# nanoporetech/bonito

Hardware: AMD Instinct MI355X
Metric: signal samples/sec/GPU (chunk=10000, batch=512) + read accuracy vs ref (higher is better)
Workload: dtype f16

## Files before the change

bonito_amd/_lib.py:

```python
import ctypes as C
import os

_HERE = os.path.dirname(os.path.abspath(__file__))
LIB_PATH = os.environ.get("BONITO_HIP_LIB") or os.path.join(_HERE, "libbonito_hip.so")


class HipEngineError(RuntimeError):
    """An entry point of libbonito_hip.so reported an error."""


class bh_layer_t(C.Structure):
    _fields_ = [
        ("kind", C.c_int32), ("in_size", C.c_int32), ("out_size", C.c_int32),
        ("winlen", C.c_int32), ("stride", C.c_int32), ("padding", C.c_int32),
        ("activation", C.c_int32), ("reverse", C.c_int32),
        ("nhead", C.c_int32), ("dim_ff", C.c_int32), ("win_left", C.c_int32), ("win_right", C.c_int32),
        ("scale_factor", C.c_int32), ("groups", C.c_int32), ("add_residual", C.c_int32), ("quantize", C.c_int32), ("reserved_i", C.c_int32 * 1),
        ("scale", C.c_float), ("clamp_lo", C.c_float), ("clamp_hi", C.c_float),
        ("blank_score", C.c_float), ("alpha", C.c_float), ("eps", C.c_float), ("reserved_f", C.c_float * 2),
        ("w0", C.c_void_p), ("b0", C.c_void_p), ("w1", C.c_void_p), ("b1", C.c_void_p),
        ("w2", C.c_void_p), ("w3", C.c_void_p), ("w4", C.c_void_p), ("w5", C.c_void_p),
    ]


BH_ACT = {None: 0, "none": 0, "swish": 1, "tanh": 2, "relu": 3}
BH_LAYER_CONV, BH_LAYER_LSTM, BH_LAYER_LINEAR_CRF, BH_LAYER_CLAMP = 1, 2, 3, 4
BH_LAYER_TRANSFORMER, BH_LAYER_UPSAMPLE, BH_LAYER_TCS_BLOCK, BH_LAYER_CTC_DECODER = 5, 6, 7, 8
BH_LAYER_DWCONV, BH_LAYER_RESIDUAL_PROJ, BH_LAYER_LINEAR = 9, 10, 11

_vp, _i, _f, _l, _sz = C.c_void_p, C.c_int, C.c_float, C.c_long, C.c_size_t

SIGNATURES = {
    "bh_last_error": (C.c_char_p, []),
    "bh_abi_version": (_i, []),
    "bh_sizeof_layer": (_sz, []),
    "bh_device_count": (_i, []),
    "bh_encoder_create": (_i, [C.POINTER(bh_layer_t), _i, _i, _i, _i, C.POINTER(_vp)]),
    "bh_encoder_destroy": (None, [_vp]),
    "bh_encoder_output_shape": (_i, [_vp, _i, C.POINTER(_i), C.POINTER(_i), C.POINTER(_i)]),
    "bh_encoder_forward": (_i, [_vp, _vp, _i, _i, _vp, _vp]),
    "bh_encoder_check": (_i, [_vp, _vp]),
    "bh_encoder_error_flag": (_i, [_vp]),
    "bh_encoder_last_ticket": (_l, [_vp]),
    "bh_encoder_error_flag_at": (_i, [_vp, _l]),
    "bh_encoder_ack": (_i, [_vp, _l]),
    "bh_encoder_describe": (_i, [_vp, C.c_char_p, _sz]),
    "bh_encoder_profile": (_i, [_vp, _i]),
    "bh_encoder_profile_read": (_i, [_vp, C.POINTER(C.c_float), C.POINTER(_i)]),
    "bh_crf_viterbi_workspace": (_sz, [_i, _i, _i]),
    "bh_crf_viterbi": (_i, [_vp, _i, _i, _i, _i, _f, _l, _l, _vp, _vp, _vp, _vp, _vp]),
    "bh_crf_reverse_complement": (_i, [_vp, _vp, _i, _i, _i, _i, _l, _l, _vp]),
    "bh_crf_logz": (_i, [_vp, _i, _i, _i, _f, _vp, _vp, _vp]),
    "bh_crf_seq_workspace": (_sz, [_i, _i, _i, _i]),
    "bh_crf_seq_logz": (_i, [_vp, _i, _i, _i, _i, _f, _l, _l, _vp, _i, _i, _vp, _vp, _vp, _vp]),
    "bh_crf_seq_viterbi": (_i, [_vp, _i, _i, _i, _i, _f, _l, _l, _vp, _i, _i, _vp, _vp, _vp, _vp, _vp]),
    "bh_crf_seq_logz_free": (_i, [_vp, _i, _i, _i, _f, _l, _l, _vp, _i, _i, _vp, _vp, _vp, _vp]),
    "bh_crf_logz_dense": (_i, [_vp, _i, _i, _i, _i, _f, _l, _l, _vp, _vp]),
    "bh_crf_seq_grad_workspace": (_sz, [_i, _i, _i, _i]),
    "bh_crf_seq_logz_grad": (_i, [_vp, _i, _i, _i, _i, _f, _l, _l, _vp, _i, _i, _vp, _vp, _vp, _vp, _vp, _l, _l, _i, _i, _vp]),
    "bh_crf_logz_dense_grad_workspace": (_sz, [_i, _i, _i]),
    "bh_crf_logz_dense_grad": (_i, [_vp, _i, _i, _i, _i, _f, _l, _l, _vp, _vp, _vp, _vp, _l, _l, _i, _vp]),
    "bh_sw_workspace": (_sz, [_i, _i, _i]),
    "bh_sw_align": (_i, [_vp, _l, _vp, _vp, _l, _vp, _i, _i, _i, _i, _i, _vp, _sz, _vp, _vp, _l, _vp, _vp]),
    "bh_sg_align": (_i, [_vp, _l, _vp, _vp, _l, _vp, _i, _i, _i, _i, _i, _vp, _sz, _vp, _vp, _l, _vp, _vp]),
    "bh_nw_workspace": (_sz, [_i, _i, _i, _l]),
    "bh_nw_align": (_i, [_vp, _l, _vp, _vp, _l, _vp, _i, _i, _vp, _sz, _vp, _vp, _l, _vp, _vp]),
    "bh_set_option": (_i, [C.c_char_p, _i]),
    "bh_signal_normalise": (_i, [_vp, _vp, _vp, _vp, _i, _i, C.c_double, C.c_double, C.c_double, C.c_double, C.c_double, C.c_double,
                            _i, _vp, _vp, _vp, _vp, _vp]),
    "bh_signal_chunks": (_i, [_vp, _vp, _vp, _vp, _vp, _vp, _vp, _vp, _vp, _vp, _i, _i, _vp, _vp]),
    "bh_crf_posterior_viterbi_workspace": (_sz, [_i, _i, _i]),
    "bh_crf_posterior_viterbi": (_i, [_vp, _i, _i, _i, _f, _vp, _vp, _vp, _vp]),
    "bh_beam_search_workspace": (_sz, [_i, _i, _i]),
    "bh_beam_search": (_i, [_vp, _i, _i, _i, _i, _f, _f, _f, _f, _vp, _vp, _vp, _vp, _vp, _vp]),
    "bh_beam_search_plan": (_i, [_i, _i, _i, _i, _i, C.POINTER(C.c_int32), _i]),
    "bh_linear": (_i, [_vp, _vp, _vp, _vp, _i, _i, _i, _i, _i, _i, _i, _f, _f, _f, _i, _i, _l, _l, _i, _vp]),
    "bh_linear_residual": (_i, [_vp, _vp, _vp, _vp, _i, _i, _i, _i, _i, _i, _i, _f, _f, _f, _i, _i, _l, _l, _i, _vp, _i, _f, _vp]),
    "bh_linear_qkv_rotary": (_i, [_vp, _vp, _vp, _vp, _i, _i, _i, _vp, _i, _f, _vp]),
    "bh_linear_last_kernel": (_i, []),
    "bh_conv1d_first": (_i, [_vp, _vp, _vp, _vp, _i, _i, _i, _i, _i, _i, _i, _f, _f, _l, _l, _vp]),
    "bh_conv1d_packed_halves": (_sz, [_i, _i, _i]),
    "bh_conv1d_pack": (_i, [_vp, _i, _i, _i, _vp]),
    "bh_conv1d": (_i, [_vp, _vp, _vp, _vp, _i, _i, _i, _i, _i, _i, _i, _i, _f, _f, _l, _l, _vp]),
    "bh_conv1d_front3": (_i, [_vp, _i, _i, _vp, _vp, _i, _i, _i, _f, _f, _vp, _vp, _i, _i, _i, _f, _f, _vp, _vp, _i, _i, _i, _i, _i, _f, _f,
                              _vp, _l, _l, _vp]),
    "bh_conv1d_last_kernel": (_i, []),
    "bh_ctc_greedy_decode": (_i, [_vp, _vp, _i, _i, _f, _f, _vp, _vp, _vp, _vp, _vp]),
    "bh_ctc_beam_search_workspace": (_sz, [_l, _i, _i, _i]),
    "bh_ctc_beam_search": (_i, [_vp, _vp, _i, _i, _i, _f, _vp, _vp, _vp, _vp, _vp]),
    "bh_dwconv1d": (_i, [_vp, _vp, _vp, _i, _i, _i, _i, _i, _i, _vp]),
    "bh_rotary_table": (_i, [_i, _i, _vp]),
    "bh_attention": (_i, [_vp, _vp, _vp, _i, _i, _i, _i, _i, _i, _vp]),
    "bh_attention_prerotated": (_i, [_vp, _vp, _i, _i, _i, _i, _i, _i, _vp]),
    "bh_rmsnorm_residual": (_i, [_vp, _vp, _vp, _vp, _l, _i, _f, _f, _vp]),
    "bh_lstm_pack_whh": (_i, [_vp, _i, _vp]),
    "bh_host_compact": (_l, [_vp, _l, _vp]),
    "bh_host_chunk_rows": (_l, [_vp, _l, _i, _i, _l, _l, _vp]),
    "bh_host_format_read": (_l, [_vp, _vp, _vp, _vp, _i, _l, _l, _i, _i, _i, _i, _i, _i, C.c_double, C.c_char_p, C.c_char_p, _l, _l,
                                 _vp, _l, _vp, _vp]),
    "bh_host_mean_qscore": (C.c_double, [C.c_char_p, _l]),
    "bh_host_svb16_decode": (_l, [_vp, _l, _l, _vp]),
    "bh_lstm_workspace": (_sz, [_i, _i]),
    "bh_lstm_layer": (_i, [_vp, _vp, _vp, _i, _i, _i, _i, _vp, _vp, _i, _vp]),
    "bh_lstm_q8_layer": (_i, [_vp, _f, _vp, _vp, _vp, _i, _i, _i, _i, _i, _vp, _vp, _vp, _vp]),
    "bh_lstm_layer_family": (_i, [_vp, _vp, _vp, _vp, _i, _i, _i, _i, _i, _i, _vp, _vp]),
    "bh_lstm_launch_plan": (_i, [_i, _i, _i, _i, _i, C.POINTER(C.c_int32), _i]),
    "bh_encoder_debug_read": (_i, [_vp, _vp, _sz, _sz]),
    "bh_encoder_set_option": (_i, [_vp, C.c_char_p, _i]),
}

_lib = None


CONV_KERNELS = {"none": 0, "first": 1, "ws_384": 20, "ws_96": 21, "front3_384": 30, "front3_96": 31, "dwconv": 40, "igemm_base": 100}


def conv_igemm_code(ntt, fs):
    return CONV_KERNELS["igemm_base"] + 10 * ntt + int(fs)


LSTM_FAMILIES = {"wave": 0, "fused": 1, "stream": 2, "wgx": 3, "wgx2": 4, "cta": 5, "wide": 6, "q8": 7}


def lib():
    global _lib
    if _lib is None:
        if not os.path.exists(LIB_PATH):
            raise HipEngineError(
                "%s not found: the MI355X engine is not built (run `python build.py`). "
                "bonito_amd has no CPU fallback." % LIB_PATH
            )
        import torch
        handle = C.CDLL(LIB_PATH)
        for name, (res, args) in SIGNATURES.items():
            fn = getattr(handle, name)
            fn.restype = res
            fn.argtypes = args
        if handle.bh_sizeof_layer() != C.sizeof(bh_layer_t):
            raise HipEngineError("bh_layer_t layout mismatch between include/bonito_hip.h and bonito_amd/_lib.py")
        _lib = handle
    return _lib


def last_error():
    msg = lib().bh_last_error()
    return msg.decode() if msg else ""


def check(rc, what=""):
    if rc != 0:
        raise HipEngineError("%s failed (rc=%d): %s" % (what or "libbonito_hip call", rc, last_error()))


def stream_ptr(device=None):
    import torch
    return C.c_void_p(torch.cuda.current_stream(device).cuda_stream)


def ptr(t):
    if t is None:
        return None
    return C.c_void_p(t.data_ptr())
```

bonito_amd/csrc/gemm.hip:

```cpp
#include <type_traits>
#include "common.h"
#include "kernels.h"
#include "options.h"

namespace bh {

struct GemmArgs {
    const half_t* X;
    const half_t* W;
    const float* bias;
    const half_t* res;
    int ldres;
    float res_scale = 1.0f;
    half_t* out;
    int M, N, K;
    int ldx, ldw, ldo;
    float scale;
    float clamp_lo, clamp_hi;
    int row_div;
    long row_s_hi, row_s_lo;
    int row_lim;
    int n_ft, n_tt;
    int stagger = 0;
    const float* rot_cs = nullptr;
// ... 766 lines not shown
                        for (int r = 0; r < 4; ++r) {
                            x[tt][t][r] = lo[r] * cc[r] - hi[r] * ss[r];
                            x[tt][t + 2][r] = hi[r] * cc[r] + lo[r] * ss[r];
                        }
                    }
                }
            }
        }
        if constexpr (ACT != ACT_NONE) {
#pragma unroll
            for (int tt = 0; tt < 2; ++tt)
#pragma unroll
                for (int jj = 0; jj < 4; ++jj)
#pragma unroll
                    for (int r = 0; r < 4; ++r) x[tt][jj][r] = apply_act<ACT>(x[tt][jj][r]);
        }
        if constexpr (!plain) {
#pragma unroll
            for (int tt = 0; tt < 2; ++tt)
#pragma unroll
                for (int jj = 0; jj < 4; ++jj)
#pragma unroll
                    for (int r = 0; r < 4; ++r) x[tt][jj][r] = fminf(fmaxf(x[tt][jj][r] * p.scale, p.clamp_lo), p.clamp_hi);
        }
#pragma unroll
        for (int tt = 0; tt < 2; ++tt) {
            const int r = 16 * tt + c16, sw = (c16 >> 1) & 7;
#pragma unroll
            for (int jj = 0; jj < 4; ++jj)
                *(uint2_t*)(base + r * 128 + (((2 * jj + (g >> 1)) ^ sw) << 4) + 8 * (g & 1)) =
                    __builtin_bit_cast(uint2_t, __builtin_convertvector(x[tt][jj], half4_t));
        }
    };
    auto blocks = [&](auto masked, auto with_bias) {
        constexpr bool MASKED = decltype(masked)::value;
        write_block(0, with_bias);
#pragma unroll
        for (int b = 0; b < 8; ++b) {
            const int i = b >> 1, P = b & 1;
            uint4_t o[4];
#pragma unroll
            for (int rr = 0; rr < 4; ++rr) {
                const int row = tl + 8 * rr;
                o[rr] = *(const uint4_t*)(scratch + (b & 1) * 4096 + row * 128 + ((q ^ ((row >> 1) & 7)) << 4));
            }
            if (b + 1 < 8) write_block(b + 1, with_bias);
#pragma unroll
            for (int rr = 0; rr < 4; ++rr) {
                const int u = 4 * b + rr;
                const bool live = !MASKED || tw + 32 * i + 8 * rr + tl < mlim;
                if constexpr (!MASKED) { if (u >= W4_NOW16) park[u - W4_NOW16] = o[rr]; }
                if ((!MASKED && u < W4_NOW16) || (MASKED && live))
                    __builtin_amdgcn_raw_buffer_store_b128(o[rr], orsrc, ovoff + P * 128 + (32 * i + 8 * rr) * rowbytes, 0, 0);
            }
        }
    };
    if (tw + 128 <= mlim) {
        if (p.bias != nullptr) blocks(std::false_type{}, std::true_type{});
        else blocks(std::false_type{}, std::false_type{});
        return true;
    }
    blocks(std::true_type{}, std::true_type{});
    return false;
}

template <bool GATED, bool T16, typename PARK, int NP>
__device__ __forceinline__ void w4_store_parked(const PARK (&park)[NP], const W4Store& st) {
    const __amdgpu_buffer_rsrc_t rsrc = __builtin_amdgcn_make_buffer_rsrc(
        (void*)(((unsigned long long)st.srd[1] << 32) | st.srd[0]), 0, 0x7ffffff0, 0x00020000);
    if constexpr (GATED && T16) {
#pragma unroll
        for (int idx = 0; idx < NP; ++idx) __builtin_amdgcn_raw_buffer_store_b128(park[idx], rsrc, st.voff + w4_store_rowg(idx) * st.rowb, 0, 0);
        return;
    } else {
#pragma unroll
    for (int idx = 0; idx < NP; ++idx) {
        const int row = T16 ? w4_store_row16(idx) : w4_store_row(idx), col = T16 ? w4_store_col16(idx) : w4_store_col(idx);
        if constexpr (GATED) __builtin_amdgcn_raw_buffer_store_b64(park[idx], rsrc, st.voff + col * 64 + row * st.rowb, 0, 0);
        else __builtin_amdgcn_raw_buffer_store_b128(park[idx], rsrc, st.voff + col * 128 + row * st.rowb, 0, 0);
    }
    }
}

template <int IDX0, int S, bool WIDE, bool FIRST, typename PARK>
__device__ __forceinline__ void w4_inst_st(float16_t (&acc)[4][4], half8_t (&fa)[2][4], half8_t (&fb)[2][4], const unsigned (&rab)[4],
                                           const unsigned (&rbb)[4], unsigned sa, unsigned sb, unsigned san, unsigned sbn, const unsigned (&vd1)[8],
                                           const unsigned (&vd2)[8], const char* sd1, const char* sd2, unsigned md1, unsigned md2, unsigned,
                                           const PARK (&park)[W4_NPARK], const W4Store& st, std::false_type) {
    if constexpr (S == 4 && WIDE && !FIRST) gemm_ktile_st4w<IDX0>(acc, fa, fb, rab, rbb, sa, sb, san, sbn, vd1, vd2, sd1, sd2, md1, md2, park, st.srd, st.voff, st.rowb);
    else if constexpr (S == 4 && WIDE && FIRST) gemm_ktile_first_st4w<IDX0>(acc, fa, fb, rab, rbb, sa, sb, san, sbn, vd1, vd2, sd1, sd2, md1, md2, park, st.srd, st.voff, st.rowb);
    else if constexpr (S == 4 && !WIDE && !FIRST) gemm_ktile_st4n<IDX0>(acc, fa, fb, rab, rbb, sa, sb, san, sbn, vd1, vd2, sd1, sd2, md1, md2, park, st.srd, st.voff, st.rowb);
    else if constexpr (S == 4 && !WIDE && FIRST) gemm_ktile_first_st4n<IDX0>(acc, fa, fb, rab, rbb, sa, sb, san, sbn, vd1, vd2, sd1, sd2, md1, md2, park, st.srd, st.voff, st.rowb);
    else static_assert(S == 4, "tools/gen_gemmstep.py emits the four-stores-per-instance variants only");
}

template <int IDX0, int S, bool WIDE, bool FIRST>
__device__ __forceinline__ void w4_inst_st(float4_t (&acc)[8][8], half8_t (&fa)[8], half8_t (&fb)[2][8], const unsigned (&rab)[2],
                                           const unsigned (&rbb)[2], unsigned sa, unsigned sb, unsigned san, unsigned sbn, const unsigned (&vd1)[8],
                                           const unsigned (&vd2)[8], const char* sd1, const char* sd2, unsigned md1, unsigned md2, unsigned wv,
                                           const uint4_t (&park)[W4_NPARKG], const W4Store& st, std::true_type ) {
    static_assert(S == 4, "tools/gen_gemmstep.py emits the four-stores-per-instance variants only");
    if constexpr (!FIRST) gemm_ktile16_st4g<IDX0>(acc, fa, fb, rab, rbb, sa, sb, san, sbn, vd1, vd2, sd1, sd2, md1, md2, wv, park, st.srd, st.voff, st.rowb);
    else gemm_ktile16_first_st4g<IDX0>(acc, fa, fb, rab, rbb, sa, sb, san, sbn, vd1, vd2, sd1, sd2, md1, md2, wv, park, st.srd, st.voff, st.rowb);
}
template <int IDX0, int S, bool WIDE, bool FIRST, typename PARK>
__device__ __forceinline__ void w4_inst_st(float4_t (&acc)[8][8], half8_t (&fa)[8], half8_t (&fb)[2][8], const unsigned (&rab)[2],
                                           const unsigned (&rbb)[2], unsigned sa, unsigned sb, unsigned san, unsigned sbn, const unsigned (&vd1)[8],
                                           const unsigned (&vd2)[8], const char* sd1, const char* sd2, unsigned md1, unsigned md2, unsigned wv,
                                           const PARK (&park)[W4_NPARK16], const W4Store& st, std::false_type) {
    if constexpr (S == 4 && WIDE && !FIRST) gemm_ktile16_st4w<IDX0>(acc, fa, fb, rab, rbb, sa, sb, san, sbn, vd1, vd2, sd1, sd2, md1, md2, wv, park, st.srd, st.voff, st.rowb);
    else if constexpr (S == 4 && WIDE && FIRST) gemm_ktile16_first_st4w<IDX0>(acc, fa, fb, rab, rbb, sa, sb, san, sbn, vd1, vd2, sd1, sd2, md1, md2, wv, park, st.srd, st.voff, st.rowb);
    else if constexpr (S == 4 && !WIDE && !FIRST) gemm_ktile16_st4n<IDX0>(acc, fa, fb, rab, rbb, sa, sb, san, sbn, vd1, vd2, sd1, sd2, md1, md2, wv, park, st.srd, st.voff, st.rowb);
    else if constexpr (S == 4 && !WIDE && FIRST) gemm_ktile16_first_st4n<IDX0>(acc, fa, fb, rab, rbb, sa, sb, san, sbn, vd1, vd2, sd1, sd2, md1, md2, wv, park, st.srd, st.voff, st.rowb);
    else static_assert(S == 4, "tools/gen_gemmstep.py emits the four-stores-per-instance variants only");
}

__device__ __forceinline__ void w4_settle(float16_t (&acc)[4][4]) {
    asm volatile("s_nop 7\n\ts_nop 7\n\ts_nop 3"
                 : "+a"(acc[0][0]), "+a"(acc[0][1]), "+a"(acc[0][2]), "+a"(acc[0][3]), "+a"(acc[1][0]), "+a"(acc[1][1]), "+a"(acc[1][2]),
                   "+a"(acc[1][3]), "+a"(acc[2][0]), "+a"(acc[2][1]), "+a"(acc[2][2]), "+a"(acc[2][3]), "+a"(acc[3][0]), "+a"(acc[3][1]),
                   "+a"(acc[3][2]), "+a"(acc[3][3]));
}
__device__ __forceinline__ void w4_settle(float4_t (&acc)[8][8]) {
#define W4_ROW(i) "+a"(acc[i][0]), "+a"(acc[i][1]), "+a"(acc[i][2]), "+a"(acc[i][3]), "+a"(acc[i][4]), "+a"(acc[i][5]), "+a"(acc[i][6]), "+a"(acc[i][7])
    asm volatile("s_nop 7\n\ts_nop 7\n\ts_nop 3" : W4_ROW(0), W4_ROW(1), W4_ROW(2), W4_ROW(3), W4_ROW(4), W4_ROW(5), W4_ROW(6), W4_ROW(7));
#undef W4_ROW
}
__device__ __forceinline__ void w4_ktile(float16_t (&acc)[4][4], half8_t (&fa)[2][4], half8_t (&fb)[2][4], const unsigned (&rab)[4], const unsigned (&rbb)[4],
                                         unsigned sa, unsigned sb, unsigned san, unsigned sbn, const unsigned (&vd1)[8], const unsigned (&vd2)[8],
                                         const char* sd1, const char* sd2, unsigned md1, unsigned md2, unsigned, bool first) {
    if (first) gemm_ktile_first(acc, fa, fb, rab, rbb, sa, sb, san, sbn, vd1, vd2, sd1, sd2, md1, md2);
    else gemm_ktile(acc, fa, fb, rab, rbb, sa, sb, san, sbn, vd1, vd2, sd1, sd2, md1, md2);
}
__device__ __forceinline__ void w4_ktile(float4_t (&acc)[8][8], half8_t (&fa)[8], half8_t (&fb)[2][8], const unsigned (&rab)[2], const unsigned (&rbb)[2],
                                         unsigned sa, unsigned sb, unsigned san, unsigned sbn, const unsigned (&vd1)[8], const unsigned (&vd2)[8],
                                         const char* sd1, const char* sd2, unsigned md1, unsigned md2, unsigned wv, bool first) {
    if (first) gemm_ktile16_first(acc, fa, fb, rab, rbb, sa, sb, san, sbn, vd1, vd2, sd1, sd2, md1, md2, wv);
    else gemm_ktile16(acc, fa, fb, rab, rbb, sa, sb, san, sbn, vd1, vd2, sd1, sd2, md1, md2, wv);
}

template <int ACT, bool GATED, int S, int MODE, bool T16 = false>
__global__ __launch_bounds__(256, 1) void gemm_w4_kernel(GemmArgs p) {
    extern __shared__ __attribute__((aligned(16))) char smem[];
    const int tid = threadIdx.x;
    const int lane = tid & 63;
    const int wave = __builtin_amdgcn_readfirstlane(tid >> 6);
    const int wa = wave >> 1, wb = wave & 1;
    const int nk = p.K / 64;

    unsigned rab[T16 ? 2 : 4], rbb[T16 ? 2 : 4];
    if constexpr (T16) {
        const int row = lane & 15, kg = lane >> 4, g = (row >> 1) & 7;
#pragma unroll
        for (int sl = 0; sl < 2; ++sl) {
            const unsigned off = (unsigned)(row * 128 + (((4 * sl + kg) ^ g) << 4));
            rab[sl] = wa * 16384 + off;
            rbb[sl] = wb * 16384 + off;
        }
    } else {
        const int row = lane & 31, hh = lane >> 5, g = (row >> 1) & 7;
#pragma unroll
        for (int ks = 0; ks < 4; ++ks) {
            const unsigned off = (unsigned)(row * 128 + (((2 * ks + hh) ^ g) << 4));
            rab[ks] = wa * 16384 + off;
            rbb[ks] = wb * 16384 + off;
        }
    }
    const unsigned wdma = wave * 8192;
    const char* const Ab = (const char*)p.X;
    const char* const Bb = (const char*)p.W;

    const int GF = p.w4_gf, GT = 32 / GF;
    const int tq = p.n_tt >> 3, tr = p.n_tt & 7;
    const int nbt = ((tq + (tr ? 1 : 0)) + GT - 1) / GT, nfg = (p.n_ft + GF - 1) / GF;
    const int slots = 8 * nfg * nbt * 32;
    auto tile_of = [&](int w, int& f0, int& t0) -> bool {
        const int xcd = w & 7, loc = w >> 3;
        const int NT = tq + (xcd < tr ? 1 : 0), tlo = xcd * tq + min(xcd, tr);
        const int blk = loc >> 5, within = loc & 31;
        const int fg = p.w4_order ? blk % nfg : blk / nbt, tg = p.w4_order ? blk / nfg : blk - fg * nbt;
        const int tf = fg * GF + within % GF, tt = tg * GT + within / GF;
        f0 = tf * 256;
        t0 = (tlo + tt) * 256;
        return tf < p.n_ft && tt < NT;
    };
    auto next_valid = [&](int w, int& f0, int& t0) -> int {
        for (; w < slots; w += gridDim.x)
            if (tile_of(w, f0, t0)) return w;
        return slots;
    };

    int f0 = 0, t0 = 0;
    int work = next_valid(blockIdx.x, f0, t0);
    if (work >= slots) return;
    if (p.stagger > 0) {
        const unsigned long long until = __builtin_readcyclecounter() + (unsigned long long)(((blockIdx.x >> 3) & 7) * p.stagger);
        while (__builtin_readcyclecounter() < until) __builtin_amdgcn_s_sleep(32);
    }
    unsigned va[8], vb[8];
    w4_offsets<T16>(p, f0, t0, wave, lane, va, vb);

    unsigned a0 = 0, a1 = W4_OP, a2 = 2 * W4_OP;
    unsigned b0 = W4_BRING, b1 = W4_BRING + W4_OP;
#pragma unroll
    for (int n = 0; n < 8; ++n) w4_dma(a0 + wdma + n * 1024, va[n], Ab);
#pragma unroll
    for (int n = 0; n < 8; ++n) w4_dma(b0 + wdma + n * 1024, vb[n], Bb);
#pragma unroll
    for (int n = 0; n < 8; ++n) w4_dma(a1 + wdma + n * 1024, va[n], Ab + 128);
#pragma unroll
    for (int n = 0; n < 8; ++n) w4_dma(b1 + wdma + n * 1024, vb[n], Bb + 128);
    asm volatile("s_waitcnt vmcnt(16)\n\ts_barrier" ::: "memory");
    std::conditional_t<T16, half8_t[8], half8_t[2][4]> fa;
    std::conditional_t<T16, half8_t[2][8], half8_t[2][4]> fb;
    if constexpr (T16) {
        asm volatile("ds_read_b128 %0, %10 offset:0\n\tds_read_b128 %1, %10 offset:2048\n\t"
                     "ds_read_b128 %2, %11 offset:0\n\tds_read_b128 %3, %11 offset:2048\n\tds_read_b128 %4, %11 offset:4096\n\tds_read_b128 %5, %11 offset:6144\n\t"
                     "ds_read_b128 %6, %11 offset:8192\n\tds_read_b128 %7, %11 offset:10240\n\tds_read_b128 %8, %11 offset:12288\n\tds_read_b128 %9, %11 offset:14336\n\t"
                     "s_waitcnt lgkmcnt(0)"
                     : "=&v"(fa[0]), "=&v"(fa[1]), "=&v"(fb[0][0]), "=&v"(fb[0][1]), "=&v"(fb[0][2]), "=&v"(fb[0][3]), "=&v"(fb[0][4]), "=&v"(fb[0][5]),
                       "=&v"(fb[0][6]), "=&v"(fb[0][7])
                     : "v"(rab[0] + a0), "v"(rbb[0] + b0)
                     : "memory");
    } else {
    asm volatile("ds_read_b128 %0, %8 offset:0\n\tds_read_b128 %1, %8 offset:4096\n\tds_read_b128 %2, %8 offset:8192\n\tds_read_b128 %3, %8 offset:12288\n\t"
                 "ds_read_b128 %4, %9 offset:0\n\tds_read_b128 %5, %9 offset:4096\n\tds_read_b128 %6, %9 offset:8192\n\tds_read_b128 %7, %9 offset:12288\n\t"
                 "s_waitcnt lgkmcnt(0)"
                 : "=&v"(fa[0][0]), "=&v"(fa[0][1]), "=&v"(fa[0][2]), "=&v"(fa[0][3]),
                   "=&v"(fb[0][0]), "=&v"(fb[0][1]), "=&v"(fb[0][2]), "=&v"(fb[0][3])
                 : "v"(rab[0] + a0), "v"(rbb[0] + b0)
                 : "memory");
    }

#ifdef BH_GEMM_STATS
    unsigned long long st_loop = 0, st_epi = 0, st_tiles = 0;
    const unsigned long long st_t0 = __builtin_readcyclecounter(), st_r0 = __builtin_amdgcn_s_memrealtime();
#endif
    constexpr bool G16 = GATED && T16;
    using park_t = std::conditional_t<GATED && !T16, uint2_t, uint4_t>;
    constexpr int NPARK = G16 ? W4_NPARKG : T16 ? W4_NPARK16 : W4_NPARK;
    constexpr int NST = (NPARK + S - 1) / S;
    park_t park[NPARK];
    W4Store pst;
    bool parked = false;
    const char* dA = Ab + 256;
    const char* dB = Bb + 256;
    while (true) {
#ifdef BH_GEMM_STATS
        const unsigned long long st_a = __builtin_readcyclecounter();
#endif
        int nf0 = f0, nt0 = t0;
        int tf0 = 0, tt0 = 0;
        const int next = next_valid(work + gridDim.x, tf0, tt0);
        if (next < slots) { nf0 = tf0; nt0 = tt0; }
        std::conditional_t<T16, float4_t[8][8], float16_t[4][4]> acc;
#define W4_ROTATE() do { const unsigned ta = a0; a0 = a1; a1 = a2; a2 = ta; const unsigned tb = b0; b0 = b1; b1 = tb; dA += 128; dB += 128; } while (0)
#define W4_CURSOR(k) do { if ((k) == nk - 2) { int lc = lane; asm volatile("" : "+v"(lc));  \
                                               w4_offsets<T16>(p, nf0, nt0, wave, lc, va, vb); dA = Ab; dB = Bb; } } while (0)
#define W4_ARGS acc, fa, fb, rab, rbb, a0, b0, a1, b1, va, vb, dA, dB, a2 + wdma, b0 + wdma, (unsigned)wave
        if (parked) {
#define W4_ST(T) if constexpr ((T) < NST) { W4_CURSOR(T); w4_inst_st<(T) * S, S, !GATED, (T) == 0>(W4_ARGS, park, pst, std::bool_constant<G16>{}); W4_ROTATE(); }
            W4_ST(0) W4_ST(1) W4_ST(2) W4_ST(3) W4_ST(4) W4_ST(5) W4_ST(6) W4_ST(7)
#undef W4_ST
            for (int k = NST; k < nk; ++k) {
                W4_CURSOR(k);
                w4_ktile(W4_ARGS, false);
                W4_ROTATE();
            }
        } else {
            w4_ktile(W4_ARGS, true);
            W4_ROTATE();
            for (int k = 1; k < nk; ++k) {
                W4_CURSOR(k);
                w4_ktile(W4_ARGS, false);
                W4_ROTATE();
            }
        }
#undef W4_ARGS
#undef W4_CURSOR
#undef W4_ROTATE
#ifdef BH_GEMM_STATS
        const unsigned long long st_b = __builtin_readcyclecounter();
#endif
        w4_settle(acc);
        if constexpr (G16) parked = w4_epilogue16g(p, acc, f0, t0, wa, wb, lane, smem + a2 + wdma, park, pst);
        else if constexpr (T16 && (MODE & 1) == 0) parked = w4_epilogue16p<ACT, MODE>(p, acc, f0, t0, wa, wb, lane, smem + a2 + wdma, park, pst);
        else parked = w4_epilogue<ACT, GATED, MODE>(p, acc, f0, t0, wa, wb, lane, smem + a2 + wdma, park, pst);
#ifdef BH_GEMM_STATS
        st_loop += st_b - st_a; st_epi += __builtin_readcyclecounter() - st_b; ++st_tiles;
#endif
        if (next >= slots) break;
        work = next; f0 = nf0; t0 = nt0;
    }
    if (parked) w4_store_parked<GATED, T16>(park, pst);
    asm volatile("s_waitcnt vmcnt(0)" ::: "memory");
#ifdef BH_GEMM_STATS
    if (p.dbg != nullptr && tid == 0 && (blockIdx.x == 0 || blockIdx.x == 133)) {
        unsigned long long* d = p.dbg + (blockIdx.x == 0 ? 0 : 8);
        d[0] = st_loop; d[1] = st_epi; d[2] = __builtin_readcyclecounter() - st_t0; d[3] = __builtin_amdgcn_s_memrealtime() - st_r0; d[4] = st_tiles;
    }
#endif
}

#ifdef BH_GEMM_STATS
unsigned long long* g_gemm_dbg = nullptr;
#endif
static int g_last_kernel = 0;

enum GemmKernel : int { GEMM_V1 = 1, GEMM_V2 = 2, GEMM_V3 = 3, GEMM_W4_T32 = 5, GEMM_W4_T16 = 6 };
enum GemmPath : int {
    PATH_AUTO = 0,
    PATH_V1_ONLY = 1,
    PATH_NO_256 = 2,
    PATH_NO_W4 = 3,
    PATH_FORCE_W4 = 5
};

#define W4_INSTANCES(X)                                                                                                  \
    X(ACT_NONE, true, 0)                                                                                                 \
    X(ACT_NONE, false, 0) X(ACT_NONE, false, 1) X(ACT_NONE, false, 2) X(ACT_NONE, false, 4)                              \
    X(ACT_TANH, false, 4) X(ACT_TANH, false, 0)                                                                          \
    X(ACT_SWISH, false, 0)
constexpr int w4_key(int act, bool gated, int mode) { return (act << 4) | (gated ? 8 : 0) | mode; }
static int w4_mode(const GemmArgs& a) {
    const bool plain = a.scale == 1.0f && a.clamp_lo == -INFINITY && a.clamp_hi == INFINITY;
    return (a.res != nullptr ? 1 : 0) | (a.rot_cs != nullptr ? 2 : 0) | (plain ? 0 : 4);
}
static bool w4_has_instance(int act, bool gated, int mode) {
    switch (w4_key(act, gated, mode)) {
#define W4_CASE(A_, G_, MODE_) case w4_key(A_, G_, MODE_):
        W4_INSTANCES(W4_CASE)
#undef W4_CASE
        return true;
    }
    return false;
}

static bool enough_tiles_256(const GemmArgs& a) { return (long)((a.N + BF3 - 1) / BF3) * ((a.M + BT3 - 1) / BT3) >= 512; }
static bool offsets_fit_256(const GemmArgs& a) { return (long)a.M * a.ldx < (1l << 31) && (long)a.N * a.ldw < (1l << 31); }
static bool shape_allows_w4(const GemmArgs& a) {
    return a.K % 128 == 0 && a.K >= 384
           && a.N % 256 == 0
           && ((a.row_div == 1 && a.row_s_hi == 1) || a.row_div % 256 == 0)
           && (a.rot_cs == nullptr || a.rot_T >= 256)
           && (long)a.ldo * 2 * (a.row_div == 1 ? 1 : a.row_s_lo) < (1l << 24)
           && offsets_fit_256(a);
}
static bool shape_allows_v3(const GemmArgs& a) {
    return a.K % BK3 == 0
           && a.N >= 256 && a.N % 16 == 0
           && offsets_fit_256(a);
}
static bool shape_allows_v2(const GemmArgs& a) { return a.K % BK2 == 0; }

static bool path_permits(int path, GemmKernel family) {
    switch (family) {
        case GEMM_W4_T32: case GEMM_W4_T16: return path == PATH_AUTO || path == PATH_FORCE_W4;
        case GEMM_V3: return path == PATH_AUTO || path == PATH_NO_W4;
        case GEMM_V2: return path != PATH_V1_ONLY;
        default: return true;
    }
}

struct GemmPlan {
    GemmKernel kernel;
    int grid, block, lds;
    int mode;
    GemmArgs args;
};
static GemmPlan gemm_plan(const GemmArgs& a, int act, bool gated, const Options& opt, int cus) {
    GemmPlan p;
    p.args = a;
    p.mode = w4_mode(a);
    const int path = opt.gemm_path;
    const bool w4 = shape_allows_w4(a) && (enough_tiles_256(a) || path == PATH_FORCE_W4) && path_permits(path, GEMM_W4_T16) &&
                    w4_has_instance(act, gated, p.mode);
    const bool v3 = !w4 && shape_allows_v3(a) && enough_tiles_256(a) && path_permits(path, GEMM_V3);
    if (!w4 && !v3) {
        p.kernel = shape_allows_v2(a) && path_permits(path, GEMM_V2) ? GEMM_V2 : GEMM_V1;
        p.grid = a.n_ft * a.n_tt; p.block = 256; p.lds = p.kernel == GEMM_V2 ? 4 * TILE2 : 4 * TILE_BYTES;
        return p;
    }
    const int nf = (a.N + BF3 - 1) / BF3, nt = (a.M + BT3 - 1) / BT3;
    p.args.n_ft = nf; p.args.n_tt = nt;
    if (v3) {
        p.kernel = GEMM_V3;
        p.args.stagger = opt.gemm_stagger;
        p.grid = nf * nt < cus ? nf * nt : cus; p.block = 512; p.lds = 4 * TILE3;
        return p;
    }
    p.kernel = opt.gemm_tile16 ? GEMM_W4_T16 : GEMM_W4_T32;
    p.args.stagger = opt.gemm_stagger > 0 ? opt.gemm_stagger * 256 : 0;
    p.args.w4_order = opt.gemm_order;
    int gf = 4;
    if (opt.gemm_gf > 0) for (gf = 32; gf > opt.gemm_gf;) gf >>= 1;
    while (gf > 1 && (gf > nf || (opt.gemm_gf <= 0 && nf % gf != 0))) gf >>= 1;
    p.args.w4_gf = gf;
    const int gt = 32 / gf, ntx = (nt >> 3) + ((nt & 7) ? 1 : 0);
    const long slots = 8l * ((nf + gf - 1) / gf) * ((ntx + gt - 1) / gt) * 32;
    p.grid = slots < cus ? (int)slots : cus; p.block = 256; p.lds = W4_LDS;
    return p;
}

template <int ACT, bool GATED, int MODE, bool T16>
static int launch_w4_instance(const GemmPlan& p, hipStream_t s) {
    BH_CHECK_HIP(bh_max_lds((const void*)gemm_w4_kernel<ACT, GATED, 4, MODE, T16>, p.lds));
    hipLaunchKernelGGL((gemm_w4_kernel<ACT, GATED, 4, MODE, T16>), dim3(p.grid), dim3(p.block), p.lds, s, p.args);
    return 0;
}
template <int ACT, bool GATED>
static int launch_w4(const GemmPlan& p, hipStream_t s) {
    switch (w4_key(ACT, GATED, p.mode)) {
#define W4_CASE(A_, G_, MODE_)                                                                                                   \
    case w4_key(A_, G_, MODE_):                                                                                                  \
        if constexpr (ACT == A_ && GATED == G_)                                                                                  \
            return p.kernel == GEMM_W4_T16 ? launch_w4_instance<ACT, GATED, MODE_, true>(p, s) : launch_w4_instance<ACT, GATED, MODE_, false>(p, s); \
        break;
        W4_INSTANCES(W4_CASE)
#undef W4_CASE
    }
    BH_REQUIRE(false, "linear: gemm_w4_kernel has no instance for activation %d, gated %d, mode %d", ACT, (int)GATED, p.mode);
}

template <int ACT, bool GATED>
static int launch(const GemmArgs& a, hipStream_t s) {
    const GemmPlan p = gemm_plan(a, ACT, GATED, g_opt, bh_cu_count());
    switch (p.kernel) {
        case GEMM_W4_T32: case GEMM_W4_T16:
            if (int rc = launch_w4<ACT, GATED>(p, s)) return rc;
            break;
        case GEMM_V3:
            BH_CHECK_HIP(bh_max_lds((const void*)gemm_big_kernel<ACT, GATED>, p.lds));
            hipLaunchKernelGGL((gemm_big_kernel<ACT, GATED>), dim3(p.grid), dim3(p.block), p.lds, s, p.args);
            break;
        case GEMM_V2:
            hipLaunchKernelGGL((gemm_glds_kernel<ACT, GATED>), dim3(p.grid), dim3(p.block), p.lds, s, p.args);
            break;
        case GEMM_V1:
            hipLaunchKernelGGL((gemm_kernel<ACT, GATED>), dim3(p.grid), dim3(p.block), p.lds, s, p.args);
            break;
    }
    g_last_kernel = p.kernel;
    return 0;
}

static GemmArgs gemm_args(const void* X, const void* W, const float* bias, void* out, int M, int N, int K, int ldx, int ldw, int ldo) {
    GemmArgs a;
    a.X = (const half_t*)X; a.W = (const half_t*)W; a.bias = bias; a.out = (half_t*)out;
    a.res = nullptr; a.ldres = 0;
    a.M = M; a.N = N; a.K = K; a.ldx = ldx; a.ldw = ldw; a.ldo = ldo;
    a.scale = 1.0f; a.clamp_lo = -INFINITY; a.clamp_hi = INFINITY;
    a.row_div = 1; a.row_s_hi = 1; a.row_s_lo = 0; a.row_lim = 0x7fffffff;
    a.n_ft = (N + BF - 1) / BF; a.n_tt = (M + BT - 1) / BT;
#ifdef BH_GEMM_STATS
    a.dbg = g_gemm_dbg;
#endif
    return a;
}

}

int bh_k_linear_last_kernel() { return bh::g_last_kernel; }

int bh_k_linear(const void* X, const void* W, const float* bias, void* out, int M, int N, int K,
                int ldx, int ldw, int ldo, int act, float scale, float clamp_lo, float clamp_hi,
                int gated, int row_div, long row_s_hi, long row_s_lo, int row_lim, hipStream_t stream,
                const void* residual, int ldres, float res_scale) {
    using namespace bh;
    BH_REQUIRE(M > 0 && N > 0 && K > 0, "linear: empty problem M=%d N=%d K=%d", M, N, K);
    BH_REQUIRE(K % 8 == 0 && ldx % 8 == 0 && ldw % 8 == 0, "linear: K/ldx/ldw must be multiples of 8 halves");
    BH_REQUIRE(ldo % 8 == 0, "linear: ldo must be a multiple of 8 halves");
    BH_REQUIRE(!gated || (N % 16 == 0), "linear: gated epilogue needs N %% 16 == 0");
    BH_REQUIRE(residual == nullptr || ldres % 8 == 0, "linear: ldres must be a multiple of 8 halves");
    GemmArgs a = gemm_args(X, W, bias, out, M, N, K, ldx, ldw, ldo);
    a.res = (const half_t*)residual; a.ldres = ldres; a.res_scale = res_scale;
    a.scale = scale; a.clamp_lo = clamp_lo; a.clamp_hi = clamp_hi;
    if (row_div > 0) {
        a.row_div = row_div; a.row_s_hi = row_s_hi; a.row_s_lo = row_s_lo;
        if (row_lim > 0) a.row_lim = row_lim;
    }
    int rc = 0;
    if (gated) { rc = launch<ACT_NONE, true>(a, stream); }
    else switch (act) {
        case ACT_NONE: rc = launch<ACT_NONE, false>(a, stream); break;
        case ACT_SWISH: rc = launch<ACT_SWISH, false>(a, stream); break;
        case ACT_TANH: rc = launch<ACT_TANH, false>(a, stream); break;
        case ACT_RELU: rc = launch<ACT_RELU, false>(a, stream); break;
        default: BH_REQUIRE(false, "linear: unknown activation %d", act);
    }
    if (rc) return rc;
    BH_CHECK_HIP(hipGetLastError());
    return 0;
}

int bh_k_linear_qkv_rotary(const void* X, const void* W, const float* bias, void* out, int M, int D, int K, const float* cos_sin,
                           int T, float qscale, hipStream_t stream) {
    using namespace bh;
    BH_REQUIRE(M > 0 && D > 0 && K > 0 && T > 0 && cos_sin != nullptr, "linear_qkv_rotary: bad arguments");
    BH_REQUIRE(D % 64 == 0 && K % 8 == 0, "linear_qkv_rotary: d_model must be a multiple of 64 (heads of 64), K of 8");
    GemmArgs a = gemm_args(X, W, bias, out, M, 3 * D, K, K, K, 3 * D);
    a.rot_cs = cos_sin; a.rot_T = T; a.rot_nfeat = 2 * D; a.rot_qfeat = D; a.rot_qscale = qscale;
    if (int rc = launch<ACT_NONE, false>(a, stream)) return rc;
    BH_CHECK_HIP(hipGetLastError());
    return 0;
}
```

bonito_amd/csrc/options.cpp:

```cpp
#include "options.h"

#include <string.h>

namespace bh {

Options g_opt;

#define BH_OPT(name) #name, &Options::name
static constexpr OptionRow OPTION_TABLE[] = {
    {BH_OPT(gemm_path), 0, Norm::keep, "linear GEMM kernel families: 0 auto, 1 = v1 only, 2 = no 256-tile kernel, 3 = no four-wave kernel, 5 = four-wave wherever legal"},
    {BH_OPT(gemm_tile16), 1, Norm::flag, "four-wave GEMM K-tile stream: 1 = 16x16x32 MFMAs, 0 = 32x32x16 (agree to fp16 rounding)"},
    {BH_OPT(gemm_order), 1, Norm::flag, "four-wave GEMM work order in an XCD: 1 = feature groups fastest, 0 = token blocks fastest (same bytes)"},
    {BH_OPT(gemm_gf), 0, Norm::keep, "four-wave GEMM feature tiles per block: 0 automatic, else rounded down to 1 / 2 / 4 / 8 / 16 / 32 (same bytes)"},
    {BH_OPT(gemm_stagger), 0, Norm::keep, "start-phase stagger of the persistent GEMM kernels, 0 = off (same bytes; measured without effect)"},
    {BH_OPT(attn_waves), 0, Norm::keep, "ring attention waves per workgroup: 0 automatic, 8, 12 (same results)"},
    {BH_OPT(attn_version), 2, Norm::one_or_two, "ring attention kernel: 2 = current, 1 = the first ring kernel"},
    {BH_OPT(attn_expt), 0, Norm::keep, "timing experiments of the ring attention kernel (bit mask): RESULTS ARE WRONG ON PURPOSE unless 0"},
    {BH_OPT(beam_fork), -1, Norm::keep, "posterior scan next to the beam kernel on a helper stream: -1 auto, 0 never, 1 always"},
    {BH_OPT(beam_select), 0, Norm::keep, "beam top-W selection: 0 histogram + boundary ranking, 1 radix search (same beams)"},
    {BH_OPT(beam_fuse), -1, Norm::keep, "forward / posterior scan as a second wave of the beam kernel: -1 auto (<= 256 states), 0 never, 1 always"},
    {BH_OPT(beam_cpw), 0, Norm::keep, "chunks per workgroup of the fused beam kernel at 256 states: 0 automatic, 1, 2, 4 (same bytes)"},
    {BH_OPT(decode_nt), 0, Norm::keep, "non-temporal score loads in the decode scans: 0 off"},
    {BH_OPT(viterbi_quad), 1, Norm::keep, "CRF Viterbi: 1 = four states per thread where the layout allows, 0 = the one-state kernel everywhere"},
    {BH_OPT(conv_ws), 1, Norm::keep, "weight-stationary kernel for the 384- / 96-channel 19-tap convolution: 1 on, 0 = generic implicit GEMM"},
    {BH_OPT(conv_fs), 1, Norm::keep, "feature-split instances of the implicit-GEMM convolution: 1 on, 0 = position-split"},
    {BH_OPT(conv_fuse), 1, Norm::keep, "conv1 -> conv2 -> conv3 as one kernel: 1 = 384-channel stacks, 2 = also 96-channel, 0 = three kernels"},
    {BH_OPT(conv_lds_kb), 64, Norm::positive_or_def, "KiB of LDS a workgroup of the implicit-GEMM convolution may take for its input span"},
    {BH_OPT(conv_front_pipe), 1, Norm::keep, "fused front end of the 384-channel stacks: 1 = conv1 / conv2 of the next block beside conv3 (12-wave pipeline), 0 = phase after phase (same bytes)"},
    {BH_OPT(conv_front_wgs), 0, Norm::keep, "workgroups of the pipelined front end: 0 = one per CU, n > 0 caps the grid (same bytes; test hook, A/B)"},
    {BH_OPT(lstm_max_spins), 1000000, Norm::nonneg_or_def, "bound of the recurrent kernels' exchange spin loops (0: the first incomplete poll round is a timeout)"},
    {BH_OPT(lstm_q8_variant), 0, Norm::keep, "geometry of the 8-bit recurrent kernel, read at bh_encoder_create: 0, 1, 2"},
};
#undef BH_OPT

static constexpr bool defaults_agree() {
    constexpr Options o{};
    for (const OptionRow& r : OPTION_TABLE)
        if (o.*r.member != r.def) return false;
    return true;
}
static_assert(defaults_agree(), "options.h and OPTION_TABLE state different defaults");
static_assert(sizeof(OPTION_TABLE) / sizeof(OPTION_TABLE[0]) == sizeof(Options) / sizeof(int), "every member of Options has exactly one row");

const OptionRow* find_option(const char* name) {
    for (const OptionRow& r : OPTION_TABLE)
        if (!strcmp(name, r.name)) return &r;
    return nullptr;
}

}
```

bonito_amd/csrc/options.h:

```cpp
#pragma once

namespace bh {

struct Options {
    int gemm_path = 0;
    int gemm_tile16 = 1;
    int gemm_order = 1;
    int gemm_gf = 0;
    int gemm_stagger = 0;
    int attn_waves = 0;
    int attn_version = 2;
    int attn_expt = 0;
    int beam_fork = -1;
    int beam_select = 0;
    int beam_fuse = -1;
    int beam_cpw = 0;
    int decode_nt = 0;
    int viterbi_quad = 1;
    int conv_ws = 1;
    int conv_fs = 1;
    int conv_fuse = 1;
    int conv_lds_kb = 64;
    int conv_front_pipe = 1;
    int conv_front_wgs = 0;
    int lstm_max_spins = 1000000;
    int lstm_q8_variant = 0;
};
extern Options g_opt;

enum class Norm {
    keep,
    flag,
    one_or_two,
    positive_or_def,
    nonneg_or_def
};
struct OptionRow {
    const char* name;
    int Options::*member;
    int def;
    Norm norm;
    const char* what;
    int normalise(int v) const {
        switch (norm) {
            case Norm::flag: return v ? 1 : 0;
            case Norm::one_or_two: return v == 1 ? 1 : 2;
            case Norm::positive_or_def: return v > 0 ? v : def;
            case Norm::nonneg_or_def: return v >= 0 ? v : def;
            default: return v;
        }
    }
};
const OptionRow* find_option(const char* name);

}
```

Before: 441.9 million.

## Add weight-stationary persistent GEMM kernel for the K=384 CRF head

Adds a persistent kernel for the CRF head linear layer (K=384, N a multiple of 256). Each workgroup keeps a 256-feature slice of the weights in registers and streams 32-row input tiles through a 4-deep LDS ring fed by async DMA. Epilogue stores of the previous tile are interleaved with the MFMAs of the current one. It is enabled by default on the auto path for M >= 262144, with an option to fall back to the four-wave kernel. The cost is a large amount of hand-scheduled asm and tight register pressure (weights held in registers, one workgroup per CU).

```diff
diff --git a/bonito_amd/_lib.py b/bonito_amd/_lib.py
--- a/bonito_amd/_lib.py
+++ b/bonito_amd/_lib.py
@@ -119,6 +119,10 @@
     return CONV_KERNELS["igemm_base"] + 10 * ntt + int(fs)
 
 
+GEMM_KERNELS = {"none": 0, "v1": 1, "glds": 2, "big": 3, "w4_t32": 5, "w4_t16": 6, "crf_head_ws": 7}
+GEMM_PATH_FORCE_W4, GEMM_PATH_FORCE_WS = 5, 7
+
+
 LSTM_FAMILIES = {"wave": 0, "fused": 1, "stream": 2, "wgx": 3, "wgx2": 4, "cta": 5, "wide": 6, "q8": 7}
 
 
diff --git a/bonito_amd/csrc/gemm.hip b/bonito_amd/csrc/gemm.hip
--- a/bonito_amd/csrc/gemm.hip
+++ b/bonito_amd/csrc/gemm.hip
@@ -1092,18 +1092,193 @@
 #endif
 }
 
+constexpr int WS_K = 384, WS_ROWS = 32, WS_ROWB = WS_K * 2, WS_STAGE = WS_ROWS * WS_ROWB, WS_DEPTH = 4, WS_SCR = 4096;
+constexpr int WS_LDS = WS_DEPTH * WS_STAGE + 4 * WS_SCR;
+constexpr int WS_DMA = WS_STAGE / 1024 / 4;
+constexpr unsigned WS_DEAD = 0x80000000u;
+
+struct WsCursor { int st, hi, sg; };
+
+template <bool SC>
+__global__ __launch_bounds__(256, 1) void crf_head_ws_kernel(GemmArgs p) {
+    extern __shared__ __attribute__((aligned(16))) char smem[];
+    const int tid = threadIdx.x;
+    const int lane = tid & 63;
+    const int wave = __builtin_amdgcn_readfirstlane(tid >> 6);
+    const int c16 = lane & 15, g = lane >> 4;
+    const int tl = lane >> 3, q = lane & 7;
+
+    const bool ident = p.row_div == 1 && p.row_s_hi == 1;
+    const int G = ident ? p.M : p.row_div;
+    const long s_hi = ident ? 0 : p.row_s_hi, s_lo = ident ? 1 : p.row_s_lo;
+    const int glim = ident ? p.M : min(p.row_div, p.row_lim);
+    const int spg = (G + WS_ROWS - 1) / WS_ROWS, ngroups = (p.M + G - 1) / G;
+    const int NS = spg * ngroups;
+    const unsigned rowbytes = (unsigned)(s_lo * p.ldo * 2);
+
+    const int nfg = p.N >> 8, nw = gridDim.x >> 3;
+    const int xcd = blockIdx.x & 7, loc = blockIdx.x >> 3;
+    const int fg = loc % nfg, tlane = loc / nfg, ntl = nw / nfg;
+    const int s_beg = (int)((long)NS * xcd >> 3), s_end = (int)((long)NS * (xcd + 1) >> 3);
+    if (tlane >= ntl || s_beg + tlane >= s_end) return;
+    const int nst = (s_end - s_beg - tlane + ntl - 1) / ntl;
+    const int dq = ntl / spg, dr = ntl - dq * spg;
+    auto advance = [&](WsCursor& c) {
+        c.st += ntl; c.hi += dq; c.sg += dr;
+        if (c.sg >= spg) { c.sg -= spg; c.hi += 1; }
+    };
+    WsCursor first;
+    first.st = s_beg + tlane; first.hi = first.st / spg; first.sg = first.st - first.hi * spg;
+    const int fw = fg * 256 + wave * 64;
+
+    half8_t wreg[4][12];
+#pragma unroll
+    for (int j = 0; j < 4; ++j)
+#pragma unroll
+        for (int s = 0; s < 12; ++s) wreg[j][s] = *(const half8_t*)(p.W + (long)(fw + 16 * j + c16) * p.ldw + 32 * s + 8 * g);
+    float4_t bj[4];
+#pragma unroll
+    for (int j = 0; j < 4; ++j) {
+        bj[j] = float4_t{0.f, 0.f, 0.f, 0.f};
+        if (p.bias != nullptr) bj[j] = *(const float4_t*)(p.bias + fw + 16 * j + 4 * g);
+    }
+
+    int drow[WS_DMA];
+    unsigned dchunk[WS_DMA];
+#pragma unroll
+    for (int k = 0; k < WS_DMA; ++k) {
+        const int u = (wave * WS_DMA + k) * 64 + lane;
+        drow[k] = u / 48;
+        dchunk[k] = (unsigned)(((u % 48) ^ (drow[k] & 15)) << 4);
+    }
+    const unsigned xrowb = (unsigned)p.ldx * 2u;
+    auto dma_m0 = [&](const WsCursor& c) {
+        return __builtin_amdgcn_readfirstlane(min(c.st < s_end ? c.hi * G + c.sg * WS_ROWS : first.hi * G + first.sg * WS_ROWS, p.M - 1));
+    };
+    auto dma_piece = [&](int m0, int slot, int k) {
+        w4_dma((unsigned)(slot * WS_STAGE + (wave * WS_DMA + k) * 1024), (unsigned)min(drow[k], p.M - 1 - m0) * xrowb + dchunk[k],
+               (const char*)p.X + (long)m0 * p.ldx * 2);
+    };
+
+    unsigned xoff[12];
+#pragma unroll
+    for (int s = 0; s < 12; ++s) xoff[s] = (unsigned)(c16 * WS_ROWB + (((4 * s + g) ^ c16) << 4));
+    char* const scr = smem + WS_DEPTH * WS_STAGE + wave * WS_SCR;
+    const unsigned ocol = (unsigned)(16 * q);
+    const unsigned srd32[2] = {(unsigned)(WS_DEPTH * WS_STAGE + wave * WS_SCR + tl * 128 + ((q ^ (tl >> 1)) << 4)),
+                               (unsigned)(WS_DEPTH * WS_STAGE + wave * WS_SCR + tl * 128 + ((q ^ ((tl >> 1) + 4)) << 4))};
+
+    auto stage = [&](float4_t (&acc)[2][4], int slot, float4_t (&prev)[2][4], const WsCursor& pc, const WsCursor& dc, int dslot) {
+        const unsigned xs32 = (unsigned)(slot * WS_STAGE);
+        const int m0d = dma_m0(dc);
+        const int sw = (c16 >> 1) & 7;
+        const int hi = __builtin_amdgcn_readfirstlane(pc.hi), lo0 = __builtin_amdgcn_readfirstlane(pc.sg * WS_ROWS);
+        const int lim = pc.st < s_end ? min(glim, p.M - hi * G) - lo0 : 0;
+        const unsigned long long ob = (unsigned long long)(p.out + ((long)hi * s_hi + (long)lo0 * s_lo) * p.ldo + fw);
+        const __amdgpu_buffer_rsrc_t rsrc = __builtin_amdgcn_make_buffer_rsrc(
+            (void*)(((unsigned long long)(unsigned)__builtin_amdgcn_readfirstlane((int)(unsigned)(ob >> 32)) << 32) |
+                    (unsigned)__builtin_amdgcn_readfirstlane((int)(unsigned)ob)), 0, 0x7ffffff0, 0x00020000);
+        uint4_t o[4];
+        auto to_scratch = [&](int tt) {
+#pragma unroll
+            for (int j = 0; j < 4; ++j) {
+                float4_t x = prev[tt][j] + bj[j];
+                if constexpr (SC) {
+#pragma unroll
+                    for (int r = 0; r < 4; ++r) x[r] = fminf(fmaxf(x[r] * p.scale, p.clamp_lo), p.clamp_hi);
+                }
+                *(uint2_t*)(scr + (16 * tt + c16) * 128 + (((2 * j + (g >> 1)) ^ sw) << 4) + 8 * (g & 1)) =
+                    __builtin_bit_cast(uint2_t, __builtin_convertvector(x, half4_t));
+            }
+        };
+        auto store = [&](int rr) {
+            const int row = tl + 8 * rr;
+            const unsigned vo = row < lim ? (unsigned)row * rowbytes + ocol : WS_DEAD;
+            __builtin_amdgcn_raw_buffer_store_b128(o[rr], rsrc, (int)vo, 0, 0);
+        };
+        half8_t xf[3][2];
+        auto frag_read = [&](int s) {
+            asm volatile("ds_read_b128 %0, %2\n\tds_read_b128 %1, %2 offset:%3"
+                         : "=&v"(xf[s % 3][0]), "=&v"(xf[s % 3][1]) : "v"(xs32 + xoff[s]), "i"(16 * WS_ROWB) : "memory");
+        };
+        frag_read(0);
+        frag_read(1);
+#pragma unroll
+        for (int tt = 0; tt < 2; ++tt)
+#pragma unroll
+            for (int j = 0; j < 4; ++j) acc[tt][j] = float4_t{0.f, 0.f, 0.f, 0.f};
+#pragma unroll
+        for (int s = 0; s < 12; ++s) {
+            if (s == 6) {
+                frag_read(s + 2);
+                asm volatile("s_waitcnt lgkmcnt(4)" : "+v"(xf[s % 3][0]), "+v"(xf[s % 3][1]), "+v"(o[0]), "+v"(o[1]), "+v"(o[2]), "+v"(o[3])::"memory");
+            } else if (s + 2 < 12) {
+                frag_read(s + 2);
+                asm volatile("s_waitcnt lgkmcnt(4)" : "+v"(xf[s % 3][0]), "+v"(xf[s % 3][1])::"memory");
+            } else if (s + 1 < 12) {
+                asm volatile("s_waitcnt lgkmcnt(2)" : "+v"(xf[s % 3][0]), "+v"(xf[s % 3][1])::"memory");
+            } else {
+                asm volatile("s_waitcnt lgkmcnt(0)" : "+v"(xf[s % 3][0]), "+v"(xf[s % 3][1])::"memory");
+            }
+#pragma unroll
+            for (int tt = 0; tt < 2; ++tt)
+#pragma unroll
+                for (int j = 0; j < 4; ++j) acc[tt][j] = mfma16(wreg[j][s], xf[s % 3][tt], acc[tt][j]);
+            if (s == 0) to_scratch(0);
+            if (s == 2) to_scratch(1);
+            if (s == 4)
+                asm volatile(
+                    "ds_read_b128 %0, %4\n\tds_read_b128 %1, %5 offset:1024\n\tds_read_b128 %2, %4 offset:2048\n\tds_read_b128 %3, %5 offset:3072"
+                    : "=&v"(o[0]), "=&v"(o[1]), "=&v"(o[2]), "=&v"(o[3]) : "v"(srd32[0]), "v"(srd32[1]) : "memory");
+            if (s == 6) { store(0); store(1); }
+            if (s == 8) { store(2); store(3); }
+            if (s & 1) dma_piece(m0d, dslot, s >> 1);
+        }
+    };
+
+    WsCursor cd = first, cc = first, cp;
+    cp.st = s_end; cp.hi = 0; cp.sg = 0;
+#pragma unroll
+    for (int n = 0; n < WS_DEPTH - 1; ++n) {
+        const int m0 = dma_m0(cd);
+#pragma unroll
+        for (int k = 0; k < WS_DMA; ++k) dma_piece(m0, n, k);
+        advance(cd);
+    }
+    asm volatile("s_waitcnt vmcnt(0)" ::: "memory");
+    float4_t acc0[2][4], acc1[2][4];
+#pragma unroll
+    for (int tt = 0; tt < 2; ++tt)
+#pragma unroll
+        for (int j = 0; j < 4; ++j) acc1[tt][j] = float4_t{0.f, 0.f, 0.f, 0.f};
+    int slot = 0;
+    for (int n = 0; n < nst; n += 2) {
+        asm volatile("s_waitcnt vmcnt(20)\n\ts_barrier" ::: "memory");
+        stage(acc0, slot, acc1, cp, cd, (slot + 3) & 3);
+        advance(cd); cp = cc; advance(cc);
+        asm volatile("s_waitcnt vmcnt(20)\n\ts_barrier" ::: "memory");
+        stage(acc1, slot + 1, acc0, cp, cd, slot);
+        advance(cd); cp = cc; advance(cc);
+        slot ^= 2;
+    }
+    asm volatile("s_waitcnt vmcnt(0)\n\ts_barrier" ::: "memory");
+    stage(acc0, slot, acc1, cp, cd, (slot + 3) & 3);
+    asm volatile("s_waitcnt vmcnt(0)" ::: "memory");
+}
+
 #ifdef BH_GEMM_STATS
 unsigned long long* g_gemm_dbg = nullptr;
 #endif
 static int g_last_kernel = 0;
 
-enum GemmKernel : int { GEMM_V1 = 1, GEMM_V2 = 2, GEMM_V3 = 3, GEMM_W4_T32 = 5, GEMM_W4_T16 = 6 };
+enum GemmKernel : int { GEMM_V1 = 1, GEMM_V2 = 2, GEMM_V3 = 3, GEMM_W4_T32 = 5, GEMM_W4_T16 = 6, GEMM_WS = 7 };
 enum GemmPath : int {
     PATH_AUTO = 0,
     PATH_V1_ONLY = 1,
     PATH_NO_256 = 2,
     PATH_NO_W4 = 3,
-    PATH_FORCE_W4 = 5
+    PATH_FORCE_W4 = 5,
+    PATH_FORCE_WS = 7
 };
 
 #define W4_INSTANCES(X)                                                                                                  \
@@ -1136,6 +1311,12 @@
            && (long)a.ldo * 2 * (a.row_div == 1 ? 1 : a.row_s_lo) < (1l << 24)
            && offsets_fit_256(a);
 }
+static bool call_allows_ws(const GemmArgs& a, int act, bool gated, int mode, int cus) {
+    return a.K == WS_K && a.N % 256 == 0 && a.N / 256 <= cus / 8 && act == ACT_NONE && !gated && (mode & ~4) == 0
+           && (long)a.ldo * 2 * (a.row_div == 1 && a.row_s_hi == 1 ? 1 : a.row_s_lo) < (1l << 24)
+           && a.M <= 0x7fffff00 && (long)a.N * a.ldw < (1l << 31);
+}
+constexpr int WS_AUTO_MIN_ROWS = 262144;
 static bool shape_allows_v3(const GemmArgs& a) {
     return a.K % BK3 == 0
            && a.N >= 256 && a.N % 16 == 0
@@ -1163,6 +1344,12 @@
     p.args = a;
     p.mode = w4_mode(a);
     const int path = opt.gemm_path;
+    if (call_allows_ws(a, act, gated, p.mode, cus) && (path == PATH_FORCE_WS || (path == PATH_AUTO && opt.crf_head_ws && a.M >= WS_AUTO_MIN_ROWS))) {
+        p.kernel = GEMM_WS;
+        p.args.n_ft = a.N / 256; p.args.n_tt = 0;
+        p.grid = cus / 8 * 8; p.block = 256; p.lds = WS_LDS;
+        return p;
+    }
     const bool w4 = shape_allows_w4(a) && (enough_tiles_256(a) || path == PATH_FORCE_W4) && path_permits(path, GEMM_W4_T16) &&
                     w4_has_instance(act, gated, p.mode);
     const bool v3 = !w4 && shape_allows_v3(a) && enough_tiles_256(a) && path_permits(path, GEMM_V3);
@@ -1218,6 +1405,19 @@
     switch (p.kernel) {
         case GEMM_W4_T32: case GEMM_W4_T16:
             if (int rc = launch_w4<ACT, GATED>(p, s)) return rc;
+            break;
+        case GEMM_WS:
+            if constexpr (ACT == ACT_NONE && !GATED) {
+                if (p.mode & 4) {
+                    BH_CHECK_HIP(bh_max_lds((const void*)crf_head_ws_kernel<true>, p.lds));
+                    hipLaunchKernelGGL((crf_head_ws_kernel<true>), dim3(p.grid), dim3(p.block), p.lds, s, p.args);
+                } else {
+                    BH_CHECK_HIP(bh_max_lds((const void*)crf_head_ws_kernel<false>, p.lds));
+                    hipLaunchKernelGGL((crf_head_ws_kernel<false>), dim3(p.grid), dim3(p.block), p.lds, s, p.args);
+                }
+            } else {
+                BH_REQUIRE(false, "linear: crf_head_ws_kernel has no instance for activation %d, gated %d", ACT, (int)GATED);
+            }
             break;
         case GEMM_V3:
             BH_CHECK_HIP(bh_max_lds((const void*)gemm_big_kernel<ACT, GATED>, p.lds));
diff --git a/bonito_amd/csrc/options.cpp b/bonito_amd/csrc/options.cpp
--- a/bonito_amd/csrc/options.cpp
+++ b/bonito_amd/csrc/options.cpp
@@ -8,11 +8,12 @@
 
 #define BH_OPT(name) #name, &Options::name
 static constexpr OptionRow OPTION_TABLE[] = {
-    {BH_OPT(gemm_path), 0, Norm::keep, "linear GEMM kernel families: 0 auto, 1 = v1 only, 2 = no 256-tile kernel, 3 = no four-wave kernel, 5 = four-wave wherever legal"},
+    {BH_OPT(gemm_path), 0, Norm::keep, "linear GEMM kernel families: 0 auto, 1 = v1 only, 2 = no 256-tile kernel, 3 = no four-wave kernel, 5 = four-wave wherever legal, 7 = weight-stationary CRF head wherever it serves"},
     {BH_OPT(gemm_tile16), 1, Norm::flag, "four-wave GEMM K-tile stream: 1 = 16x16x32 MFMAs, 0 = 32x32x16 (agree to fp16 rounding)"},
     {BH_OPT(gemm_order), 1, Norm::flag, "four-wave GEMM work order in an XCD: 1 = feature groups fastest, 0 = token blocks fastest (same bytes)"},
     {BH_OPT(gemm_gf), 0, Norm::keep, "four-wave GEMM feature tiles per block: 0 automatic, else rounded down to 1 / 2 / 4 / 8 / 16 / 32 (same bytes)"},
     {BH_OPT(gemm_stagger), 0, Norm::keep, "start-phase stagger of the persistent GEMM kernels, 0 = off (same bytes; measured without effect)"},
+    {BH_OPT(crf_head_ws), 1, Norm::flag, "weight-stationary kernel for the CRF head (K = 384, >= 262144 rows) on the automatic path: 1 on, 0 = four-wave kernel (same bytes)"},
     {BH_OPT(attn_waves), 0, Norm::keep, "ring attention waves per workgroup: 0 automatic, 8, 12 (same results)"},
     {BH_OPT(attn_version), 2, Norm::one_or_two, "ring attention kernel: 2 = current, 1 = the first ring kernel"},
     {BH_OPT(attn_expt), 0, Norm::keep, "timing experiments of the ring attention kernel (bit mask): RESULTS ARE WRONG ON PURPOSE unless 0"},
diff --git a/bonito_amd/csrc/options.h b/bonito_amd/csrc/options.h
--- a/bonito_amd/csrc/options.h
+++ b/bonito_amd/csrc/options.h
@@ -8,6 +8,7 @@
     int gemm_order = 1;
     int gemm_gf = 0;
     int gemm_stagger = 0;
+    int crf_head_ws = 1;
     int attn_waves = 0;
     int attn_version = 2;
     int attn_expt = 0;
```

New measurement: 443.1 million, median of 6. Within noise of the previous version (+0.3%).
